# jeffreychou777/GenComm

Measured on AMD Instinct MI355X. Metric: scenes/sec, higher is better.
Workload: dtype f32

## Files before the change

gencomm_amd/csrc/conv8h8_kernels.h:

```cpp
#pragma once
#include "conv8h_kernels.h"
#include "split_f16.h"

namespace gc {

constexpr int H8_TH = 8, H8_LH = H8_TH + 2;
constexpr int H8_PLANE = H8_LH * HC_ROW;
constexpr int H8_TPLANE = H8_PLANE / 2;
constexpr int H8_TOFF = 2 * H8_PLANE;
constexpr int H8_TILE_BYTES = 2 * H8_PLANE + H8_TPLANE;

struct Tile8Regs {
  float4 v[8];
  float2 h;
};
template <bool GN>
__device__ __forceinline__ void h8_load(Tile8Regs& R, const float* __restrict__ sp, unsigned plane_in, int H, int W, int x0, int y0, int tid) {
  const int r0 = tid >> 4, qx = tid & 15;
  if (r0 < H8_LH) {
    const int gy = y0 - 1 + r0, gx = x0 + 4 * qx;
    if (GN) {
      const int cy = min(max(gy, 0), H - 1), cx = min(gx, W - 4);
#pragma unroll
      for (int c = 0; c < 8; ++c) R.v[c] = *reinterpret_cast<const float4*>(sp + ((unsigned)c * plane_in + (unsigned)cy * (unsigned)W + (unsigned)cx));
// ... 159 lines not shown
      for (int c = 0; c < 8; ++c) q = fmax(q, __hip_atomic_load(st + 2 * c + 1, __ATOMIC_RELAXED, __HIP_MEMORY_SCOPE_AGENT));
      bound = sqrtf((float)q) * 1.0001f;
    }
    mul = act_scale(bound);
  }
  const float inv_s = a.wh[NSRC * HC_WTAB3] / mul;
  const float4 bias4 = *reinterpret_cast<const float4*>(a.bias + 4 * ch);
  const float bias[4] = {bias4.x, bias4.y, bias4.z, bias4.w};
  Tile8Regs R;
  h8_load<GN>(R, a.src[0] + (size_t)n * 8 * plane, (unsigned)plane, a.H, a.W, x0, y0, tid);
  if (GN) {
    if (tid < NSRC * 8) {
      const int s = tid >> 3, c = tid & 7;
      float A, B;
      gn_coeff(a.sstat[s] + (size_t)n * 16, c, 2 * NSRC, a.inv_cnt, a.gamma[tid], a.beta[tid], &A, &B);
      s_ab[tid][0] = HC_NL2E * A;
      s_ab[tid][1] = HC_NL2E * B;
    }
    __syncthreads();
  }
  f32x4 acc[4];
  {
    const float sc = a.wh[NSRC * HC_WTAB3 + 1] * mul;
    const f32x4 b0 = {bias[0] * sc, bias[1] * sc, bias[2] * sc, bias[3] * sc};
#pragma unroll
    for (int j = 0; j < 4; ++j) acc[j] = b0;
  }
  h8_stage<GN>(tile, R, a.H, a.W, x0, y0, &s_ab[0], tid, mul);
  int off[4][3];
  h8_lane_offsets(off, wave, lane);
  float resv[RES == 1 ? 4 : 1][4];
  if (RES == 1 && wave_live) {
#pragma unroll
    for (int i = 0; i < 4; ++i) {
      const float* __restrict__ rp = a.res[0] + ((size_t)n * 8 + 4 * ch + i) * plane + (size_t)gy * a.W + gx;
      float4 r = make_float4(0.f, 0.f, 0.f, 0.f);
      if (vec_ok && gy < a.H) r = *reinterpret_cast<const float4*>(rp);
      resv[i][0] = r.x; resv[i][1] = r.y; resv[i][2] = r.z; resv[i][3] = r.w;
    }
  }
  if (NSRC == 2) h8_load<GN>(R, a.src[1] + (size_t)n * 8 * plane, (unsigned)plane, a.H, a.W, x0, y0, tid);
  __syncthreads();
  if (wave_live) h8_mfma3(tile, a.wh, acc, off, lane);
  if (NSRC == 2) {
    __syncthreads();
    h8_stage<GN>(tile, R, a.H, a.W, x0, y0, &s_ab[8], tid, 1.0f);
    __syncthreads();
    if (wave_live) h8_mfma3(tile, a.wh + HC_WTAB3, acc, off, lane);
  }
  float part[8];
#pragma unroll
  for (int i = 0; i < 8; ++i) part[i] = 0.f;
  if (wave_live) {
    float out[4][4];
#pragma unroll
    for (int i = 0; i < 4; ++i)
#pragma unroll
      for (int j = 0; j < 4; ++j) out[i][j] = RES == 1 ? fmaf(acc[j][i], inv_s, resv[i][j]) : acc[j][i] * inv_s;
    if (RES == 2) {
#pragma unroll 8
      for (int c = 0; c < 16; ++c) {
        const float4 wv4 = *reinterpret_cast<const float4*>(a.ninw + c * 8 + 4 * ch);
        const float wv[4] = {wv4.x, wv4.y, wv4.z, wv4.w};
        const float* __restrict__ rp = a.res[c >> 3] + ((size_t)n * 8 + (c & 7)) * plane + (size_t)gy * a.W + gx;
        float4 t = make_float4(0.f, 0.f, 0.f, 0.f);
        if (vec_ok && gy < a.H) t = *reinterpret_cast<const float4*>(rp);
        const float r[4] = {t.x, t.y, t.z, t.w};
#pragma unroll
        for (int i = 0; i < 4; ++i)
#pragma unroll
          for (int j = 0; j < 4; ++j) out[i][j] = fmaf(wv[i], r[j], out[i][j]);
      }
    }
#pragma unroll
    for (int i = 0; i < 4; ++i) {
      if (vec_ok && gy < a.H) {
        float* __restrict__ dp = a.dst + ((size_t)n * 8 + 4 * ch + i) * plane + (size_t)gy * a.W + gx;
        *reinterpret_cast<float4*>(dp) = make_float4(out[i][0], out[i][1], out[i][2], out[i][3]);
        float s = out[i][0] + out[i][1], q = out[i][0] * out[i][0];
        q = fmaf(out[i][1], out[i][1], q);
#pragma unroll
        for (int j = 2; j < 4; ++j) { s += out[i][j]; q = fmaf(out[i][j], out[i][j], q); }
        part[i] = s;
        part[4 + i] = q;
      }
    }
  }
  if (a.dstat != nullptr) hc_stats_commit(part, s_red, a.dstat + (size_t)n * 16, tid);
}

}
```

gencomm_amd/csrc/conv8h_kernels.h:

```cpp
#pragma once
#include "split_f16.h"
#include "unet_kernels.h"
#include "unet_plan.h"

namespace gc {

constexpr int HC_TW = 64, HC_TH = 16, HC_NT = 256, HC_LH = 18;
constexpr int HC_SLOTS = 18;
constexpr int HC_PHASE = HC_SLOTS * 16;
constexpr int HC_ROW = 4 * HC_PHASE;
constexpr int HC_PLANE = HC_LH * HC_ROW;
constexpr int HC_WTAB = 3 * 2 * 64 * 4;
constexpr int HC_WC3 = 3 * 64 * 4 + 64 * 2;
constexpr int HC_WTAB3 = 3 * HC_WC3;
static_assert(HC_WTAB3 == kWtab3, "unet_plan.h sizes the prepared blob with kWtab3");
constexpr int HC_TPLANE = HC_PLANE / 2;
constexpr int HC_TOFF = 2 * HC_PLANE;

constexpr float HC_NL2E = -1.4426950408889634f;
__device__ __forceinline__ void gn_silu_zr(float a2, float b2, float x, float& z, float& r, float cs = HC_NL2E) {
  z = fmaf(a2, x, b2);
  r = __builtin_amdgcn_rcpf(fmaf(cs, __builtin_amdgcn_exp2f(z), cs));
}
__device__ __forceinline__ int hc_addr(int row, int px ) {
// ... 390 lines not shown
    half8_t w[3];
#pragma unroll
    for (int k = 0; k < 3; ++k) w[k] = __builtin_bit_cast(half8_t, *reinterpret_cast<const uint4*>(tab + c * HC_WC3 + (k * 64 + lane) * 4));
#pragma unroll
    for (int p = 0; p < 2; ++p) {
      half8_t b[4];
#pragma unroll
      for (int j = 0; j < 4; ++j) b[j] = *reinterpret_cast<const half8_t*>(tile + off[j][c] + p * 2 * HC_ROW);
#pragma unroll
      for (int j = 0; j < 4; ++j) acc[p][j] = __builtin_amdgcn_mfma_f32_16x16x32_f16(w[2], b[j], acc[p][j], 0, 0, 0);
#pragma unroll
      for (int j = 0; j < 4; ++j) acc[p][j] = __builtin_amdgcn_mfma_f32_16x16x32_f16(w[1], b[j], acc[p][j], 0, 0, 0);
#pragma unroll
      for (int j = 0; j < 4; ++j) acc[p][j] = __builtin_amdgcn_mfma_f32_16x16x32_f16(w[0], b[j], acc[p][j], 0, 0, 0);
    }
  }
}

__device__ __forceinline__ void load_wa(half8_t (&wa)[3][2], const float* __restrict__ tab, int lane) {
#pragma unroll
  for (int c = 0; c < 3; ++c)
#pragma unroll
    for (int h = 0; h < 2; ++h) {
      const uint4 v = *reinterpret_cast<const uint4*>(tab + ((c * 2 + h) * 64 + lane) * 4);
      wa[c][h] = __builtin_bit_cast(half8_t, v);
    }
}

__device__ __forceinline__ void hc_stats_commit(float (&part)[8], float (*s_red)[16], double* __restrict__ dstat, int tid) {
  const int lane = tid & 63, wave = tid >> 6, ch = (lane >> 4) & 1;
#pragma unroll
  for (int v = 0; v < 8; ++v) {
    float x = part[v];
    x = dpp_add<0x111, 0xf>(x);
    x = dpp_add<0x112, 0xf>(x);
    x = dpp_add<0x114, 0xf>(x);
    x = dpp_add<0x118, 0xf>(x);
    x += __shfl_xor(x, 32, 64);
    part[v] = x;
  }
  if (lane == 15 || lane == 31) {
#pragma unroll
    for (int i = 0; i < 4; ++i) {
      s_red[wave][4 * ch + i] = part[i];
      s_red[wave][8 + 4 * ch + i] = part[4 + i];
    }
  }
  __syncthreads();
  if (tid < 16) {
    float v = 0.f;
#pragma unroll
    for (int w = 0; w < HC_NT / 64; ++w) v += s_red[w][tid];
    atomicAdd(&dstat[(tid & 7) * 2 + (tid >> 3)], (double)v);
  }
}

constexpr int HC_TILE_BYTES = 2 * HC_PLANE + HC_TPLANE;
struct HcCarry {
  TileRegs<HC_TW, HC_TH, HC_NT, 8> R;
  float2 hreg;
};
template <int NSRC, bool GN, bool UP, int RES, bool DIAG = false, bool PERSIST = false>
__device__ __forceinline__ void conv8h_tile(const Conv8Args& a, const BlockId bid, unsigned char* tile, float (*s_ab)[2], float (*s_red)[16],
                                            size_t bias_off, HcCarry& carry, bool have_next, const BlockId next) {
  constexpr int NT = HC_NT, TW = HC_TW, TH = HC_TH;
  TileRegs<TW, TH, NT, 8>& R = carry.R;
  float2& hreg = carry.hreg;
  fp16_ovfl_clamp();
  int tid_ = threadIdx.x;
  if (PERSIST) asm volatile("" : "+v"(tid_));
  const int tid = tid_, lane = tid & 63, wave = tid >> 6;
  const int n = bid.z;
  const int x0 = bid.x * TW, y0 = bid.y * TH;
  const size_t plane_in = (size_t)a.Hin * a.Win;
  const size_t plane = (size_t)a.H * a.W;
  const bool wvec = UP ? ((a.Win & 1) == 0) : ((a.W & 3) == 0);
  const int ln = lane & 15, g = lane >> 4, ch = g & 1, rr = g >> 1;
  const int gx = x0 + 4 * ln;
  const int gy0 = y0 + 4 * wave + rr;
  const bool vec_ok = (gx + 3 < a.W) && ((a.W & 3) == 0);
  const bool wave_live = y0 + 4 * wave < a.H;

  GC_STAMP(0);
  float mul = 1.0f;
  if (!GN) {
    float bound = 0.f;
    if (a.amax != nullptr) {
      bound = *a.amax;
    } else if (a.sstat[0] != nullptr) {
      const double* st = a.sstat[0] + (size_t)n * 16;
      double q = 0.0;
#pragma unroll
      for (int c = 0; c < 8; ++c) q = fmax(q, __hip_atomic_load(st + 2 * c + 1, __ATOMIC_RELAXED, __HIP_MEMORY_SCOPE_AGENT));
      bound = sqrtf((float)q) * 1.0001f;
    }
    mul = act_scale(bound);
  }
  const float inv_s = a.wh[NSRC * HC_WTAB3] / mul;
  const float4 bias4 = *reinterpret_cast<const float4*>(a.bias + bias_off + 4 * ch);
  const float bias[4] = {bias4.x, bias4.y, bias4.z, bias4.w};
  if (!PERSIST) {
    hreg = make_float2(0.f, 0.f);
    if (wvec) {
      stage_load<TW, TH, NT, 8, UP, GN>(R, a.src[0] + (size_t)n * 8 * plane_in, (unsigned)plane_in, a.Win, a.H, a.W, x0, y0, tid);
      hreg = halo_load_h<UP>(a.src[0] + (size_t)n * 8 * plane_in, (unsigned)plane_in, a.Win, a.H, a.W, x0, y0, tid);
    }
  }
  auto prefetch_next = [&]() {
    if (PERSIST && have_next) {
      const float* np = a.src[0] + (size_t)next.z * 8 * plane_in;
      stage_load<TW, TH, NT, 8, UP, GN>(R, np, (unsigned)plane_in, a.Win, a.H, a.W, next.x * TW, next.y * TH, tid);
      hreg = halo_load_h<UP>(np, (unsigned)plane_in, a.Win, a.H, a.W, next.x * TW, next.y * TH, tid);
    }
  };
  if (GN) {
    if (tid < NSRC * 8) {
      const int s = tid >> 3, c = tid & 7;
      float A, B;
      gn_coeff(a.sstat[s] + (size_t)n * 16, c, 2 * NSRC, a.inv_cnt, a.gamma[tid], a.beta[tid], &A, &B);
      s_ab[tid][0] = HC_NL2E * A;
      s_ab[tid][1] = HC_NL2E * B;
    }
    __syncthreads();
  }

  GC_STAMP(1);
  f32x4 acc[2][4];
  const float bsc = a.wh[NSRC * HC_WTAB3 + 1] * mul;
  const f32x4 b0 = {bias[0] * bsc, bias[1] * bsc, bias[2] * bsc, bias[3] * bsc};
  if (DIAG || !wave_live) {
#pragma unroll
    for (int p = 0; p < 2; ++p)
#pragma unroll
      for (int j = 0; j < 4; ++j) acc[p][j] = b0;
  }

  if (wvec) stage_store_h<GN, true>(tile, R, hreg, a.H, a.W, x0, y0, &s_ab[0], tid, mul);
  else stage_tile_scalar_h<GN, UP, true>(tile, a.src[0] + (size_t)n * 8 * plane_in, (unsigned)plane_in, a.Win, a.H, a.W, x0, y0, &s_ab[0], tid, mul);
  int off[4][3];
  hc_lane_offsets(off, wave, lane);
  float resv[RES == 1 ? 2 : 1][4][4];
  auto request_residual = [&]() {
  if (RES == 1 && wave_live) {
    const float* const lane_res = a.res[0] + ((size_t)n * 8 + 4 * ch) * plane + (size_t)gy0 * a.W + gx;
#pragma unroll
    for (int p = 0; p < 2; ++p)
#pragma unroll
      for (int i = 0; i < 4; ++i) {
        const int gy = gy0 + 2 * p;
        const float* __restrict__ rp = lane_res + ((size_t)i * plane + (size_t)(2 * p) * a.W);
        if (vec_ok && gy < a.H) {
          const float4 r = *reinterpret_cast<const float4*>(rp);
          resv[p][i][0] = r.x; resv[p][i][1] = r.y; resv[p][i][2] = r.z; resv[p][i][3] = r.w;
        } else {
#pragma unroll
          for (int j = 0; j < 4; ++j) resv[p][i][j] = (gy < a.H && gx + j < a.W) ? rp[j] : 0.f;
        }
      }
  }
  };
  constexpr bool LATE2 = PERSIST;
  auto early = [&]() {
    if (!PERSIST) request_residual();
    if (NSRC == 2 && wvec && !LATE2) {
      stage_load<TW, TH, NT, 8, UP, GN>(R, a.src[1] + (size_t)n * 8 * plane_in, (unsigned)plane_in, a.Win, a.H, a.W, x0, y0, tid);
      hreg = halo_load_h<UP>(a.src[1] + (size_t)n * 8 * plane_in, (unsigned)plane_in, a.Win, a.H, a.W, x0, y0, tid);
    }
  };
#ifdef HC_EARLY_IN_FRONT
  early();
#endif
  __syncthreads();
  GC_STAMP(2);
#ifdef HC_PRIO_MFMA
  __builtin_amdgcn_s_setprio(HC_PRIO_MFMA);
#endif
#ifdef HC_EARLY_IN_FRONT
  if (wave_live) conv_tile_mfma3<DIAG, NSRC == 2 && (!LATE2 || PERSIST), !DIAG>(tile, a.wh, acc, off, lane, a.term_mask, b0);
#else
  if (wave_live) conv_tile_mfma3<DIAG, NSRC == 2 && (!LATE2 || PERSIST), !DIAG>(tile, a.wh, acc, off, lane, a.term_mask, b0, early);
  else early();
#endif
  if (NSRC == 2 && wvec && LATE2) {
    stage_load<TW, TH, NT, 8, UP, GN>(R, a.src[1] + (size_t)n * 8 * plane_in, (unsigned)plane_in, a.Win, a.H, a.W, x0, y0, tid);
    hreg = halo_load_h<UP>(a.src[1] + (size_t)n * 8 * plane_in, (unsigned)plane_in, a.Win, a.H, a.W, x0, y0, tid);
  }
  if (DIAG && (a.term_mask & 128) && wave_live) conv_tile_mfma3<DIAG, NSRC == 2>(tile, a.wh, acc, off, lane, a.term_mask);
  GC_STAMP(3);
  if (NSRC == 2) {
    __syncthreads();
    if (wvec) stage_store_h<GN, true>(tile, R, hreg, a.H, a.W, x0, y0, &s_ab[8], tid);
    else stage_tile_scalar_h<GN, UP, true>(tile, a.src[1] + (size_t)n * 8 * plane_in, (unsigned)plane_in, a.Win, a.H, a.W, x0, y0, &s_ab[8], tid);
    __syncthreads();
    if (wave_live) conv_tile_mfma3<false, PERSIST>(tile, a.wh + HC_WTAB3, acc, off, lane);
  }

  if (PERSIST) request_residual();
  if (RES != 2) prefetch_next();
  GC_STAMP(4);
#ifdef HC_PRIO_EPI
  __builtin_amdgcn_s_setprio(HC_PRIO_EPI);
#endif
  float part[8];
#pragma unroll
  for (int i = 0; i < 8; ++i) part[i] = 0.f;
  if (wave_live) {
    float* const lane_dst = a.dst + ((size_t)n * 8 + 4 * ch) * plane + (size_t)gy0 * a.W + gx;
    float out[2][4][4];
#pragma unroll
    for (int p = 0; p < 2; ++p)
#pragma unroll
      for (int i = 0; i < 4; ++i)
#pragma unroll
        for (int j = 0; j < 4; ++j) out[p][i][j] = RES == 1 ? fmaf(acc[p][j][i], inv_s, resv[p][i][j]) : acc[p][j][i] * inv_s;

    if (RES == 2) {
      const size_t lane_off = (size_t)n * 8 * plane;
      if ((a.W & 3) == 0) {
        int gxl = gx, gyl = gy0;
        asm volatile("" : "+v"(gxl), "+v"(gyl));
        const int cx = min(gxl, a.W - 4);
        const int cy0 = min(gyl, a.H - 1), d1 = (min(gyl + 2, a.H - 1) - cy0) * a.W;
        const size_t o0 = lane_off + (size_t)cy0 * a.W + cx;
        const float* const lp[2][2] = {{a.res[0] + o0, a.res[0] + o0 + d1}, {a.res[1] + o0, a.res[1] + o0 + d1}};
        constexpr int CB = 4;
        float4 rq[2][CB][2];
        auto issue = [&](int b, int st) {
#pragma unroll
          for (int c = 0; c < CB; ++c)
#pragma unroll
            for (int p = 0; p < 2; ++p) {
              const int cc = b * CB + c;
              rq[st][c][p] = *reinterpret_cast<const float4*>(lp[cc >> 3][p] + (size_t)(cc & 7) * plane);
            }
        };
        issue(0, 0);
#pragma unroll
        for (int b = 0; b < 16 / CB; ++b) {
          __builtin_amdgcn_sched_barrier(0);
          if (b + 1 < 16 / CB) issue(b + 1, (b + 1) & 1);
#pragma unroll
          for (int c = 0; c < CB; ++c) {
            const float4 wv4 = *reinterpret_cast<const float4*>(a.ninw + (b * CB + c) * 8 + 4 * ch);
            const float wv[4] = {wv4.x, wv4.y, wv4.z, wv4.w};
#pragma unroll
            for (int p = 0; p < 2; ++p) {
              const float4 t = rq[b & 1][c][p];
              const float r[4] = {t.x, t.y, t.z, t.w};
#pragma unroll
              for (int i = 0; i < 4; ++i)
#pragma unroll
                for (int j = 0; j < 4; ++j) out[p][i][j] = fmaf(wv[i], r[j], out[p][i][j]);
            }
          }
        }
      } else {
#pragma unroll 1
        for (int c = 0; c < 16; ++c) {
          const float4 wv4 = *reinterpret_cast<const float4*>(a.ninw + c * 8 + 4 * ch);
          const float wv[4] = {wv4.x, wv4.y, wv4.z, wv4.w};
#pragma unroll
          for (int p = 0; p < 2; ++p) {
            const int gy = gy0 + 2 * p;
            const float* __restrict__ rp = a.res[c >> 3] + ((size_t)n * 8 + (c & 7)) * plane + (size_t)gy * a.W + gx;
            float r[4];
#pragma unroll
            for (int j = 0; j < 4; ++j) r[j] = (gy < a.H && gx + j < a.W) ? rp[j] : 0.f;
#pragma unroll
            for (int i = 0; i < 4; ++i)
#pragma unroll
              for (int j = 0; j < 4; ++j) out[p][i][j] = fmaf(wv[i], r[j], out[p][i][j]);
          }
        }
      }
    }

    if (RES == 2) prefetch_next();
#pragma unroll
    for (int p = 0; p < 2; ++p) {
      const int gy = gy0 + 2 * p;
#pragma unroll
      for (int i = 0; i < 4; ++i) {
        float* __restrict__ dp = lane_dst + ((size_t)i * plane + (size_t)(2 * p) * a.W);
        float s = 0.f, q = 0.f;
        if (vec_ok && gy < a.H) {
          if (!(DIAG && (a.term_mask & 64)))
            *reinterpret_cast<float4*>(dp) = make_float4(out[p][i][0], out[p][i][1], out[p][i][2], out[p][i][3]);
          s = out[p][i][0] + out[p][i][1];
          q = out[p][i][0] * out[p][i][0];
          q = fmaf(out[p][i][1], out[p][i][1], q);
#pragma unroll
          for (int j = 2; j < 4; ++j) { s += out[p][i][j]; q = fmaf(out[p][i][j], out[p][i][j], q); }
        } else {
#pragma unroll
          for (int j = 0; j < 4; ++j)
            if (gy < a.H && gx + j < a.W) { dp[j] = out[p][i][j]; s += out[p][i][j]; q = fmaf(out[p][i][j], out[p][i][j], q); }
        }
        part[i] = p == 0 ? s : part[i] + s;
        part[4 + i] = p == 0 ? q : part[4 + i] + q;
      }
    }
  } else if (RES == 2) {
    prefetch_next();
  }
  GC_STAMP(5);
  if (a.dstat != nullptr) hc_stats_commit(part, s_red, a.dstat + (size_t)n * 16, tid);
  GC_STAMP(6);
  if (PERSIST) __syncthreads();
}
template <int NSRC, bool GN, bool UP, int RES, bool DIAG = false>
__device__ __forceinline__ void conv8h_tile(const Conv8Args& a, const BlockId bid, unsigned char* tile, float (*s_ab)[2], float (*s_red)[16],
                                            size_t bias_off = 0) {
  HcCarry carry;
  conv8h_tile<NSRC, GN, UP, RES, DIAG, false>(a, bid, tile, s_ab, s_red, bias_off, carry, false, bid);
}

template <int NSRC, bool GN, bool UP, int RES, bool DIAG = false>
__global__ __launch_bounds__(HC_NT, 3) void conv8h_kernel(const Conv8Args a) {
  __shared__ __align__(16) unsigned char tile[HC_TILE_BYTES];
  __shared__ float s_ab[16][2];
  __shared__ float s_red[HC_NT / 64][16];
#ifdef HC_LDS_PAD
  __shared__ float s_pad[HC_LDS_PAD / 4];
  if (a.H < 0) s_pad[threadIdx.x] = 1.f;
#endif
  conv8h_tile<NSRC, GN, UP, RES, DIAG>(a, xcd_block(a.xcd), tile, s_ab, s_red);
}

template <int NSRC, bool GN, bool UP, int RES>
__global__ __launch_bounds__(HC_NT, 3) void conv8hp_kernel(const Conv8Args a, int tx, int ty, int nz) {
// ... 7 lines not shown
  BlockId bid = xcd_block_dims(a.xcd, lin, (unsigned)tx, (unsigned)ty, total);
  HcCarry carry;
  {
    const float* sp = a.src[0] + (size_t)bid.z * 8 * plane_in;
    stage_load<HC_TW, HC_TH, HC_NT, 8, UP, GN>(carry.R, sp, (unsigned)plane_in, a.Win, a.H, a.W, bid.x * HC_TW, bid.y * HC_TH, threadIdx.x);
    carry.hreg = halo_load_h<UP>(sp, (unsigned)plane_in, a.Win, a.H, a.W, bid.x * HC_TW, bid.y * HC_TH, threadIdx.x);
  }
#pragma unroll 1
  for (; lin < total; lin += gridDim.x) {
    const unsigned nl = lin + gridDim.x;
    const bool have_next = nl < total;
    const BlockId nb = have_next ? xcd_block_dims(a.xcd, nl, (unsigned)tx, (unsigned)ty, total) : bid;
    conv8h_tile<NSRC, GN, UP, RES, false, true>(a, bid, tile, s_ab, s_red, 0, carry, have_next, nb);
    bid = nb;
  }
}

__global__ __launch_bounds__(256) void prep_conv8h_kernel(const float* __restrict__ w, float* __restrict__ dst, int IC) {
  const int tid = threadIdx.x;
  float m = 0.f;
  for (int i = tid; i < 8 * IC * 9; i += 256) m = fmaxf(m, fabsf(w[i]));
  const float scale = block_weight_scale(m);
  const int nsrc = IC / 8;
  uint32_t* __restrict__ out = reinterpret_cast<uint32_t*>(dst);
  auto weight = [&](int s, int c, int l, int ch) -> float {
    const int mrow = l & 15, kg = l >> 4, r = mrow >> 3, oc = mrow & 7;
    const int dyp = hc_tap_row(kg), dx = c, dy = dyp - r;
    return (dy >= 0 && dy <= 2) ? w[((oc * IC + s * 8 + ch) * 3 + dy) * 3 + dx] * scale : 0.f;
  };
  for (int i = tid; i < nsrc * HC_WTAB3; i += 256) {
    const int s = i / HC_WTAB3, rem = i - s * HC_WTAB3;
    const int c = rem / HC_WC3, q = rem - c * HC_WC3;
    if (q < 768) {
      const int d = q & 3, l = (q >> 2) & 63, term = q >> 8;
      uint16_t v[2];
      for (int e = 0; e < 2; ++e) {
        const float x = weight(s, c, l, 2 * d + e);
        const _Float16 w1 = (_Float16)x;
        const float r1 = x - (float)w1;
        const _Float16 w2 = (_Float16)r1;
        const _Float16 w3 = (_Float16)(r1 - (float)w2);
        v[e] = __builtin_bit_cast(uint16_t, term == 0 ? w1 : term == 1 ? w2 : w3);
      }
      out[i] = (uint32_t)v[0] | ((uint32_t)v[1] << 16);
    } else {
      const int d = (q - 768) & 1, l = (q - 768) >> 1;
      const float k = 1.0f / HC_TSCALE;
      out[i] = bf8x4(weight(s, c, l, 4 * d) * k, weight(s, c, l, 4 * d + 1) * k, weight(s, c, l, 4 * d + 2) * k, weight(s, c, l, 4 * d + 3) * k);
    }
  }
  if (tid < 64) dst[nsrc * HC_WTAB3 + tid] = (tid & 1) ? scale : 1.0f / scale;
}

}
```

gencomm_amd/csrc/unet_host.h:

```cpp
#pragma once
#include <stdlib.h>

#include "attn_kernels.h"
#include "conv8b_kernels.h"
#include "conv8h_kernels.h"
#include "conv8h8_kernels.h"
#include "dataflow_kernels.h"
#include "latent_kernels.h"
#include "latenth_kernels.h"
#include "unet_kernels.h"
#include "unet_plan.h"

namespace gc {

inline int cdiv(int a, int b) { return (a + b - 1) / b; }

enum TileCfg { TILE_64x16 = 0, TILE_32x16 = 1, TILE_32x8 = 2 };
inline long long tile_want(const Modes& m) {
  return m.v[MODE_TILE_WANT] > 0 ? m.v[MODE_TILE_WANT] : (m.split() ? 160LL : 512LL);
}
inline TileCfg pick_tile(const Modes& m, int n, int H, int W, int zmul = 1) {
  if (m.bf16()) return TILE_64x16;
  const long long want = tile_want(m);
  if ((long long)cdiv(W, 64) * cdiv(H, 16) * n * zmul >= want) return TILE_64x16;
// ... 58 lines not shown
}

template <int NSRC, bool GN, bool UP, int RES>
inline void launch_conv8b(const Conv8BArgs& a, int n, hipStream_t st) {
  const double elt = 2.0;
  const double abytes = elt * n * ((double)NSRC * 8 * a.Hin * a.Win + (RES == 1 ? 8.0 : RES == 2 ? 16.0 : 0.0) * a.H * a.W + 8.0 * a.H * a.W);
  TimedLaunch tl(UP ? KF_UP : (NSRC == 2 ? KF_CONV16 : (RES == 1 ? KF_CONV8_RES1 : RES == 2 ? KF_CONV8_RES2 : KF_CONV8)), st, abytes);
  GC_KLOG("conv8b_kernel<...> (bf16 storage)");
  conv8b_kernel<NSRC, GN, UP, RES><<<dim3(cdiv(a.W, 64), cdiv(a.H, 16), n), 256, 0, st>>>(a);
}

struct UNetCall {
  const UNetPlan* plan;
  const UNetWorkspace* ws;
  const float* prepared;
  char* wsp;
  int n, H, W;
  hipStream_t st;
  Modes m;
  float* amax() const { return reinterpret_cast<float*>(wsp + ws->amax_off); }
  int is_f32(int id) const { return (!m.bf16() || id == plan->hs0_tensor) ? 1 : 0; }

  float* tensor_ptr(int id) const {
    const TensorPlan& t = plan->tensors[id];
    return reinterpret_cast<float*>(wsp + ws->level_base[t.level] + ws->slot_bytes[t.level] * t.slot);
  }
  double* stat_ptr(int id) const { return reinterpret_cast<double*>(wsp) + (size_t)id * n * 16; }
};

inline Conv8Args conv1_args(const UNetCall& c, const Op& o, int t) {
  const ResBlockPlan& b = c.plan->blocks[o.blk];
  const float* P = c.prepared;
  const int Hl = c.ws->Hl[o.level], Wl = c.ws->Wl[o.level];
  Conv8Args a{};
  a.src[0] = c.tensor_ptr(o.src[0]); a.sstat[0] = c.stat_ptr(o.src[0]);
  if (o.src[1] >= 0) { a.src[1] = c.tensor_ptr(o.src[1]); a.sstat[1] = c.stat_ptr(o.src[1]); }
  a.gamma = P + b.n1w; a.beta = P + b.n1b;
  a.w = P + b.p_c1w; a.wh = P + b.p_c1wh; a.bias = P + b.p_bias1 + (size_t)t * 8;
  a.dst = c.tensor_ptr(o.dst); a.dstat = c.stat_ptr(o.dst);
  a.H = a.Hin = Hl; a.W = a.Win = Wl;
  a.inv_cnt = 1.0 / ((b.cin == 8 ? 2.0 : 4.0) * Hl * Wl);
  a.xcd = c.m.xcd();
  return a;
}
inline Conv8Args conv2_args(const UNetCall& c, const Op& o) {
  const ResBlockPlan& b = c.plan->blocks[o.blk];
  const float* P = c.prepared;
  const int Hl = c.ws->Hl[o.level], Wl = c.ws->Wl[o.level];
  Conv8Args a{};
  a.src[0] = c.tensor_ptr(o.src[0]); a.sstat[0] = c.stat_ptr(o.src[0]);
  a.gamma = P + b.n2w; a.beta = P + b.n2b;
  a.w = P + b.p_c2w; a.wh = P + b.p_c2wh; a.bias = P + b.p_bias2;
  a.res[0] = c.tensor_ptr(o.res[0]);
  if (o.res[1] >= 0) { a.res[1] = c.tensor_ptr(o.res[1]); a.ninw = P + b.p_ninw; }
  a.dst = c.tensor_ptr(o.dst); a.dstat = c.stat_ptr(o.dst);
  a.H = a.Hin = Hl; a.W = a.Win = Wl;
  a.inv_cnt = 1.0 / (2.0 * Hl * Wl);
  a.xcd = c.m.xcd();
  return a;
}
inline Conv8Args up_args(const UNetCall& c, const Op& o) {
  const UNetPlan& p = *c.plan;
  const float* P = c.prepared;
  const int lin = o.level + 1;
  Conv8Args a{};
  a.src[0] = c.tensor_ptr(o.src[0]);
  a.sstat[0] = c.stat_ptr(o.src[0]);
  a.w = P + p.up[lin].p_w; a.wh = P + p.up[lin].p_wh; a.bias = P + p.up[lin].b;
  a.dst = c.tensor_ptr(o.dst); a.dstat = c.stat_ptr(o.dst);
  a.H = c.ws->Hl[o.level]; a.W = c.ws->Wl[o.level]; a.Hin = c.ws->Hl[lin]; a.Win = c.ws->Wl[lin];
  a.xcd = c.m.xcd();
  return a;
}
inline DownArgs down_args(const UNetCall& c, const Op& o) {
  const UNetPlan& p = *c.plan;
  const float* P = c.prepared;
  const int lin = o.level - 1;
  return DownArgs{c.tensor_ptr(o.src[0]), P + p.down[lin].p_w, P + p.down[lin].b, c.tensor_ptr(o.dst), c.stat_ptr(o.dst),
                  c.ws->Hl[o.level], c.ws->Wl[o.level], c.ws->Hl[lin], c.ws->Wl[lin], !c.is_f32(o.src[0]), !c.is_f32(o.dst)};
}

inline bool resfuse_emulated(const UNetCall& c, const ResBlockPlan& b, TileCfg tc, bool wvec) {
  return c.m.v[MODE_RESFUSE_EMU] != 0 && b.cin == 8 && tc == TILE_64x16 && c.m.split() && !c.m.bf16() && wvec;
}

inline bool df_eligible(const UNetCall& c, int f, int l) {
  if (c.m.v[MODE_DATAFLOW] == 0 || !c.m.split() || c.m.bf16() || l - f < 2 || l - f > DF_MAX_OPS || c.n > 64 * 1024) return false;
  if (c.m.v[MODE_CONV8H_MASK] != -1) return false;
  for (int oi = f; oi < l; ++oi) {
    const Op& o = c.plan->ops[oi];
    if (o.kind != OP_RES_CONV1 && o.kind != OP_RES_CONV2 && o.kind != OP_DOWN && o.kind != OP_UP) return false;
    if (o.kind == OP_DOWN) {
      if ((c.ws->Wl[o.level - 1] & 3) != 0) return false;
    } else if (pick_tile(c.m, c.n, c.ws->Hl[o.level], c.ws->Wl[o.level]) != TILE_64x16) return false;
  }
  return true;
}
inline int df_enqueue(const UNetCall& c, int t, int f, int l, bool upload) {
  const UNetPlan& p = *c.plan;
  DfProgram* dprog = reinterpret_cast<DfProgram*>(c.wsp + c.ws->df_prog_off);
  unsigned* words = reinterpret_cast<unsigned*>(c.wsp + c.ws->df_words_off);
  const int nops = l - f;
  if (upload) {
    static thread_local DfProgram hp;
    hp.nops = nops; hp.n = c.n;
    int qlen[8] = {0, 0, 0, 0, 0, 0, 0, 0};
    for (int k = 0; k < nops; ++k) {
// ... 249 lines not shown
  a.a_bf16 = !c.is_f32(p.last_body_tensor);
  TimedLaunch tl(KF_LATENT_STEP, c.st, 4.0 * c.n * 32.0 * c.H * c.W);
  const bool small_h = c.m.split() && (c.W & 3) == 0 && c.W >= 64 && c.H >= 16 && c.m.v[MODE_TILE_WANT] == 0;
  if ((pick_tile(c.m, c.n, c.H, c.W) == TILE_64x16 || small_h) && c.m.split()) {
    const dim3 grid(cdiv(c.W, 64), cdiv(c.H, 16), c.n);
    GC_KLOG(noise ? "latent_step_h_kernel<1> (explicit noise)" : "latent_step_h_kernel<2> (in-kernel Philox)");
    if (noise) latent_step_h_kernel<1><<<grid, 256, 0, c.st>>>(a);
    else latent_step_h_kernel<2><<<grid, 256, 0, c.st>>>(a);
  } else if (pick_tile(c.m, c.n, c.H, c.W) == TILE_64x16) {
    const dim3 grid(cdiv(c.W, 64), cdiv(c.H, 16), c.n);
    GC_KLOG(noise ? "latent_step_kernel<64,16,1> (exact fp32, explicit noise)" : "latent_step_kernel<64,16,2> (exact fp32, in-kernel Philox)");
    if (noise) latent_step_kernel<64, 16, 1><<<grid, 256, 0, c.st>>>(a);
    else latent_step_kernel<64, 16, 2><<<grid, 256, 0, c.st>>>(a);
  } else {
    const dim3 grid(cdiv(c.W, 32), cdiv(c.H, 16), c.n);
    GC_KLOG(noise ? "latent_step_kernel<32,16,1> (exact fp32, explicit noise)" : "latent_step_kernel<32,16,2> (exact fp32, in-kernel Philox)");
    if (noise) latent_step_kernel<32, 16, 1><<<grid, 128, 0, c.st>>>(a);
    else latent_step_kernel<32, 16, 2><<<grid, 128, 0, c.st>>>(a);
  }
  GC_HIP(hipGetLastError());
  return GC_OK;
}

inline int unet_prepare_enqueue(const UNetPlan& p, const float* raw, float* prepared, hipStream_t st) {
  GC_HIP(hipMemcpyAsync(prepared, raw, (size_t)p.raw_floats * sizeof(float), hipMemcpyDeviceToDevice, st));
  auto conv_w = [&](long long src, long long dst, int OC, int IC, int OCB) {
    const int total = OC * IC * 9;
    prep_conv_w_kernel<<<cdiv(total, 256), 256, 0, st>>>(raw + src, prepared + dst, OC, IC, OCB);
  };
  conv_w(p.conv_in.w, p.conv_in.p_w, 8, p.C + 2, 8);
  GC_HIP(hipMemsetAsync(prepared + p.conv_out.p_w, 0, (size_t)((p.C + 15) / 16 * 16) * 72 * sizeof(float), st));
  conv_w(p.conv_out.w, p.conv_out.p_w, p.C, 8, 16);
  prep_conv_out_h_kernel<<<1, 256, 0, st>>>(raw + p.conv_out.w, prepared + p.conv_out.p_wh, p.C);
  for (int l = 0; l < p.L; ++l) {
    if (p.down[l].w >= 0) conv_w(p.down[l].w, p.down[l].p_w, 8, 8, 8);
    if (p.up[l].w >= 0) {
      conv_w(p.up[l].w, p.up[l].p_w, 8, 8, 8);
      prep_conv8h_kernel<<<1, 256, 0, st>>>(raw + p.up[l].w, prepared + p.up[l].p_wh, 8);
      prep_conv8b_kernel<<<1, 256, 0, st>>>(raw + p.up[l].w, prepared + p.up[l].p_wb, 8);
    }
  }
  TembArgs ta{};
  ta.raw = raw; ta.prepared = prepared;
  ta.d0w = p.d0w; ta.d0b = p.d0b; ta.d1w = p.d1w; ta.d1b = p.d1b;
  ta.nblocks = (int)p.blocks.size(); ta.T = p.T;
  for (size_t i = 0; i < p.blocks.size(); ++i) {
    const ResBlockPlan& b = p.blocks[i];
    conv_w(b.c1w, b.p_c1w, 8, b.cin, 8);
    conv_w(b.c2w, b.p_c2w, 8, 8, 8);
    prep_conv8h_kernel<<<1, 256, 0, st>>>(raw + b.c1w, prepared + b.p_c1wh, b.cin);
    prep_conv8h_kernel<<<1, 256, 0, st>>>(raw + b.c2w, prepared + b.p_c2wh, 8);
    prep_conv8b_kernel<<<1, 256, 0, st>>>(raw + b.c1w, prepared + b.p_c1wb, b.cin);
    prep_conv8b_kernel<<<1, 256, 0, st>>>(raw + b.c2w, prepared + b.p_c2wb, 8);
    if (b.cin != 8) prep_nin_w_kernel<<<1, 256, 0, st>>>(raw + b.ninw, prepared + b.p_ninw, 8, b.cin);
    prep_add_kernel<<<1, 64, 0, st>>>(raw + b.c2b, b.cin != 8 ? raw + b.ninb : nullptr, prepared + b.p_bias2, 8);
    ta.tpw[i] = b.tpw; ta.tpb[i] = b.tpb; ta.c1b[i] = b.c1b; ta.dst[i] = b.p_bias1;
  }
  prep_temb_kernel<<<p.T, 64, 0, st>>>(ta);
  {
    PrepLatentArgs la{raw + p.conv_in.w, raw + p.conv_out.w, raw + p.conv_out.b, prepared + p.p_wc5, prepared + p.p_wc1,
                      prepared + p.p_bring, prepared + p.p_bsum, p.C};
    prep_latent_kernel<<<cdiv(1600 + 5184 + 72 + 8, 256), 256, 0, st>>>(la);
    prep_latent_h_kernel<<<1, 256, 0, st>>>(prepared + p.p_wc5, raw + p.conv_in.w, prepared + p.p_wc5h, prepared + p.p_wxh,
                                           prepared + p.p_wch, p.C);
  }
  GC_HIP(hipGetLastError());
  return GC_OK;
}

}
```

gencomm_amd/csrc/unet_kernels.h:

```cpp
#pragma once
#include <type_traits>

#include "common.h"

namespace gc {

__device__ __forceinline__ void gn_coeff(const double* __restrict__ stat ,
                                         int c, int gs, double inv_cnt, float gamma, float beta,
                                         float* A, float* B) {
  const int g0 = c & ~(gs - 1);
  double s = 0.0, q = 0.0;
  for (int j = 0; j < gs; ++j) {
    s += stat[(g0 + j) * 2 + 0];
    q += stat[(g0 + j) * 2 + 1];
  }
  const double mean = s * inv_cnt;
  const float var = fmaxf((float)(q * inv_cnt - mean * mean), 0.f);
  const float rstd = __builtin_amdgcn_rsqf(var + 1e-6f);
  const float a = gamma * rstd;
  *A = a;
  *B = beta - (float)mean * a;
}

template <int NT>
// ... 181 lines not shown
    constexpr int ic = decltype(IC)::value;
    float in[3][PPL + 2];
#pragma unroll
    for (int dy = 0; dy < 3; ++dy) {
      if constexpr (PPL == 4) {
        const float4 v = *reinterpret_cast<const float4*>(&tile[ic][ty + dy][tx * 4 + 4]);
        in[dy][0] = tile[ic][ty + dy][tx * 4 + 3];
        in[dy][1] = v.x; in[dy][2] = v.y; in[dy][3] = v.z; in[dy][4] = v.w;
        in[dy][5] = tile[ic][ty + dy][tx * 4 + 8];
      } else {
        in[dy][0] = tile[ic][ty + dy][tx + 3];
        in[dy][1] = tile[ic][ty + dy][tx + 4];
        in[dy][2] = tile[ic][ty + dy][tx + 5];
      }
    }
    static_for<0, 9>([&](auto TAP) {
      constexpr int tap = decltype(TAP)::value, dy = tap / 3, dx = tap % 3;
      static_for<0, NOG>([&](auto OG) {
        constexpr int og = decltype(OG)::value;
        constexpr int f = (ic * 9 + tap) * NOG + og;
#pragma unroll
        for (int p = 0; p < PPL; ++p) acc[og][p] = mfma_wbcast<f % 16>(wr[f / 16], in[dy][p + dx], acc[og][p]);
      });
    });
  });
}

__device__ __forceinline__ void gn_mean_rstd(const double* __restrict__ stat, int c, int gs, double inv_cnt, float* mean, float* rstd) {
  const int g0 = c & ~(gs - 1);
  double s = 0.0, q = 0.0;
  for (int j = 0; j < gs; ++j) { s += stat[(g0 + j) * 2 + 0]; q += stat[(g0 + j) * 2 + 1]; }
  const double m = s * inv_cnt;
  const float var = fmaxf((float)(q * inv_cnt - m * m), 0.f);
  *mean = (float)m;
  *rstd = __builtin_amdgcn_rsqf(var + 1e-6f);
}

__device__ __forceinline__ float silu_grad_f(float z) {
  const float s = sigmoid_f(z);
  return s * fmaf(z, 1.0f - s, 1.0f);
}


struct Conv8Args {
  const float* src[2];
  const double* sstat[2];
  const float* gamma;
  const float* beta;
  const float* w;
  const float* wh;
  const float* bias;
  const float* res[2];
  const float* ninw;
  float* dst;
  double* dstat;
  double inv_cnt;
  int H, W, Hin, Win;
  int xcd;
  const float* amax;
  int term_mask;
  int gn_gs;
  int src_ct, dst_ct;
};

template <int TW, int TH, int PPL, int NSRC, bool GN, bool UP, int RES>
__global__ __launch_bounds__((TW / PPL) * TH) void conv8_kernel(const Conv8Args a) {
  constexpr int NT = (TW / PPL) * TH;
  constexpr int LH = TH + 2, LS = TW + 8;
  static_assert(NT % 64 == 0, "workgroup must be whole waves");
  __shared__ __align__(16) float tile[8][LH][LS];
  __shared__ float s_ab[16][2];
  __shared__ float s_red[NT / 64][16];

  const int tid = threadIdx.x, lane = tid & 63;
  const BlockId bid = xcd_block(a.xcd);
  const int n = bid.z;
  const int x0 = bid.x * TW, y0 = bid.y * TH;
  const int tx = tid % (TW / PPL), ty = tid / (TW / PPL);
  const size_t plane_in = (size_t)a.Hin * a.Win;
  const size_t src_ns = (size_t)(a.src_ct ? a.src_ct : 8) * plane_in;
  const size_t plane = (size_t)a.H * a.W;
  const bool wvec = UP ? ((a.Win & 1) == 0) : ((a.W & 3) == 0);
  const int gy = y0 + ty, gx = x0 + tx * PPL;
  const bool row_ok = gy < a.H;
  const bool vec_ok = PPL == 4 && row_ok && (gx + 3 < a.W) && ((a.W & 3) == 0);
  bool ok[PPL];
#pragma unroll
  for (int p = 0; p < PPL; ++p) ok[p] = row_ok && (gx + p < a.W);
  const size_t pix = (size_t)gy * a.W + gx;
  constexpr int ROWS_PER_WAVE = 64 / (TW / PPL);
  const bool wave_live = y0 + (tid >> 6) * ROWS_PER_WAVE < a.H;

  GC_STAMP(0);
  float wr[NSRC][9];
#pragma unroll
  for (int s = 0; s < NSRC; ++s) load_wregs<9>(wr[s], a.w + s * 576, 576, lane);
  float bias[8];
#pragma unroll
  for (int o = 0; o < 8; ++o) bias[o] = as_const(a.bias)[o];
  TileRegs<TW, TH, NT, 8> R;
  if (GC_EXP & 16) R = TileRegs<TW, TH, NT, 8>{};
  else if (wvec) stage_load<TW, TH, NT, 8, UP>(R, a.src[0] + (size_t)n * src_ns, (unsigned)plane_in, a.Win, a.H, a.W, x0, y0, tid);
  float resv[(RES == 1 || RES == 3) ? 8 : 1][PPL];
  if (RES == 1 || RES == 3) {
#pragma unroll
    for (int o = 0; o < 8; ++o) {
// ... 575 lines not shown
```

gencomm_amd/csrc/unet_plan.h:

```cpp
#pragma once
#include <string>
#include <vector>

#include "common.h"

namespace gc {

constexpr int kWtab3 = 3 * (3 * 64 * 4 + 64 * 2);

struct ParamEntry {
  std::string name;
  long long numel;
  long long off;
};

struct ResBlockPlan {
  int cin;
  long long n1w, n1b, c1w, c1b, tpw, tpb, n2w, n2b, c2w, c2b, ninw, ninb;
  long long p_c1w, p_c2w, p_ninw, p_bias1 , p_bias2 ;
  long long p_c1wh, p_c2wh;
  long long p_c1wb, p_c2wb;
};

struct AttnPlan {
  long long nw, nb, qw, qb, kw, kb, vw, vb, pw, pb;
};

struct ConvPlan {
  long long w, b;
  long long p_w;
  long long p_wh = -1;
  long long p_wb = -1;
};

enum OpKind { OP_CONV_IN, OP_RES_CONV1, OP_RES_CONV2, OP_DOWN, OP_UP, OP_CONV_OUT, OP_ATTN };

struct Op {
  OpKind kind;
  int blk;
  int src[2];
  int res[2];
  int dst;
  int level;
};

struct TensorPlan {
  int level;
  int slot;
  int last_use;
};

struct UNetPlan {
  int C, L, R, T, attn_mask;
  std::vector<AttnPlan> attns;
  std::vector<ParamEntry> params;
  long long raw_floats = 0;
  long long prepared_floats = 0;
  long long d0w, d0b, d1w, d1b;
  ConvPlan conv_in, conv_out;
  long long nout_w, nout_b;
  long long p_wc5, p_wc1, p_bring, p_bsum;
  long long p_wc5h, p_wxh, p_wch;
  int hs0_tensor = 0, last_body_tensor = 0;
  std::vector<ConvPlan> down, up;
  std::vector<ResBlockPlan> blocks;
  std::vector<Op> ops;
  std::vector<TensorPlan> tensors;
  std::vector<int> slots_per_level;

  long long add(const std::string& name, long long numel) {
    params.push_back({name, numel, raw_floats});
    const long long o = raw_floats;
    raw_floats += numel;
    return o;
// ... 70 lines not shown
    d0b = add("temb.dense.0.bias", 32);
    d1w = add("temb.dense.1.weight", 32 * 32);
    d1b = add("temb.dense.1.bias", 32);
    conv_in.w = add("conv_in.weight", 8LL * (C + 2) * 9);
    conv_in.b = add("conv_in.bias", 8);
    std::vector<std::vector<int>> down_blk(L), up_blk(L), down_att(L), up_att(L);
    for (int l = 0; l < L; ++l) {
      for (int b = 0; b < R; ++b) {
        down_blk[l].push_back(add_resblock("down." + std::to_string(l) + ".block." + std::to_string(b), 8));
        if (attn_mask >> l & 1) down_att[l].push_back(add_attn("down." + std::to_string(l) + ".attn." + std::to_string(b)));
      }
      if (l != L - 1) {
        down[l].w = add("down." + std::to_string(l) + ".downsample.conv.weight", 8 * 8 * 9);
        down[l].b = add("down." + std::to_string(l) + ".downsample.conv.bias", 8);
      }
    }
    const int mid1 = add_resblock("mid.block_1", 8), mid2 = add_resblock("mid.block_2", 8);
    for (int l = L - 1; l >= 0; --l) {
      for (int b = 0; b <= R; ++b) {
        up_blk[l].push_back(add_resblock("up." + std::to_string(l) + ".block." + std::to_string(b), 16));
        if (attn_mask >> l & 1) up_att[l].push_back(add_attn("up." + std::to_string(l) + ".attn." + std::to_string(b)));
      }
      if (l != 0) {
        up[l].w = add("up." + std::to_string(l) + ".upsample.conv.weight", 8 * 8 * 9);
        up[l].b = add("up." + std::to_string(l) + ".upsample.conv.bias", 8);
      }
    }
    nout_w = add("norm_out.weight", 8);
    nout_b = add("norm_out.bias", 8);
    conv_out.w = add("conv_out.weight", (long long)C * 8 * 9);
    conv_out.b = add("conv_out.bias", C);
    if ((int)blocks.size() > kMaxResBlocks) return "too many res-blocks";

    prepared_floats = (raw_floats + 63) / 64 * 64;
    conv_in.p_w = padd(8LL * (C + 2) * 9);
    conv_out.p_w = padd((long long)((C + 15) / 16 * 16) * 8 * 9);
    conv_out.p_wh = padd((long long)((C + 15) / 16) * kWtab3 + 64);
    for (int l = 0; l < L; ++l) {
      if (down[l].w >= 0) down[l].p_w = padd(8 * 8 * 9);
      if (up[l].w >= 0) { up[l].p_w = padd(8 * 8 * 9); up[l].p_wh = padd(kWtab3 + 64); up[l].p_wb = padd(768); }
    }
    p_wc5 = padd(1600); p_wc1 = padd(5184); p_bring = padd(72); p_bsum = padd(8);
    p_wc5h = padd(8 * (kWtab3 / 3) + 64); p_wxh = padd((long long)(C / 8) * kWtab3); p_wch = padd(kWtab3);
    for (auto& b : blocks) {
      b.p_c1w = padd(8LL * b.cin * 9);
      b.p_c2w = padd(8 * 8 * 9);
      b.p_ninw = b.cin != 8 ? padd(8LL * b.cin) : -1;
      b.p_bias1 = padd((long long)T * 8);
      b.p_bias2 = padd(8);
      b.p_c1wh = padd((long long)(b.cin / 8) * kWtab3 + 64);
      b.p_c2wh = padd(kWtab3 + 64);
      b.p_c1wb = padd((long long)(b.cin / 8) * 768);
      b.p_c2wb = padd(768);
    }

    std::vector<int> hs;
    int h = new_tensor(0);
    ops.push_back({OP_CONV_IN, 0, {-1, -1}, {-1, -1}, h, 0});
    hs.push_back(h);
    for (int l = 0; l < L; ++l) {
      for (int b = 0; b < R; ++b) {
        int t = emit_resblock(down_blk[l][b], hs.back(), -1, l);
        if (attn_mask >> l & 1) t = emit_attn(down_att[l][b], t, l);
        hs.push_back(t);
      }
      if (l != L - 1) {
        const int d = new_tensor(l + 1);
        ops.push_back({OP_DOWN, l, {hs.back(), -1}, {-1, -1}, d, l + 1});
        hs.push_back(d);
      }
    }
    h = hs.back();
    h = emit_resblock(mid1, h, -1, L - 1);
    h = emit_resblock(mid2, h, -1, L - 1);
    for (int l = L - 1; l >= 0; --l) {
      for (int b = 0; b <= R; ++b) {
        const int skip = hs.back();
        hs.pop_back();
        h = emit_resblock(up_blk[l][b], h, skip, l);
        if (attn_mask >> l & 1) h = emit_attn(up_att[l][b], h, l);
      }
      if (l != 0) {
        const int u = new_tensor(l - 1);
        ops.push_back({OP_UP, l, {h, -1}, {-1, -1}, u, l - 1});
        h = u;
      }
    }
    ops.push_back({OP_CONV_OUT, 0, {h, -1}, {-1, -1}, -1, 0});
    hs0_tensor = ops[0].dst;
    last_body_tensor = h;

    for (int i = 0; i < (int)ops.size(); ++i) {
      const Op& o = ops[i];
      for (int k = 0; k < 2; ++k) {
        if (o.src[k] >= 0) tensors[o.src[k]].last_use = i;
        if (o.res[k] >= 0) tensors[o.res[k]].last_use = i;
      }
    }
    tensors[hs0_tensor].last_use = (int)ops.size();
    slots_per_level.assign(L, 0);
    std::vector<std::vector<int>> free_slots(L);
    auto take_slot = [&](int id) {
      TensorPlan& t = tensors[id];
      if (!free_slots[t.level].empty()) {
        t.slot = free_slots[t.level].back();
        free_slots[t.level].pop_back();
// ... 57 lines not shown
```

Before: 189.2.

## Compute nin 1x1 shortcut with split-precision MFMA instead of scalar FMAs

Replaces the scalar 16-channel 1x1 nin shortcut in the residual conv epilogue with an MFMA path. It splits activations into f16 hi/lo plus a bf8 tail and multiplies them against a prepared weight table, scaling by a bound derived from the residual tensors' statistics. A new prep kernel builds the table, and plan and args gain offsets for it and for the residual stat pointers. The goal is to offload the FMA-heavy shortcut to matrix cores and overlap next-tile prefetch with it. This adds precision-emulation error risk and extra stat reads.

Result: no change. 189.9, median of 3 (+0.4%).

```diff
diff --git a/gencomm_amd/csrc/conv8h8_kernels.h b/gencomm_amd/csrc/conv8h8_kernels.h
--- a/gencomm_amd/csrc/conv8h8_kernels.h
+++ b/gencomm_amd/csrc/conv8h8_kernels.h
@@ -235,35 +235,24 @@
 #pragma unroll
   for (int i = 0; i < 8; ++i) part[i] = 0.f;
   if (wave_live) {
-    float out[4][4];
+    float out[1][4][4];
 #pragma unroll
     for (int i = 0; i < 4; ++i)
 #pragma unroll
-      for (int j = 0; j < 4; ++j) out[i][j] = RES == 1 ? fmaf(acc[j][i], inv_s, resv[i][j]) : acc[j][i] * inv_s;
+      for (int j = 0; j < 4; ++j) out[0][i][j] = RES == 1 ? fmaf(acc[j][i], inv_s, resv[i][j]) : acc[j][i] * inv_s;
     if (RES == 2) {
-#pragma unroll 8
-      for (int c = 0; c < 16; ++c) {
-        const float4 wv4 = *reinterpret_cast<const float4*>(a.ninw + c * 8 + 4 * ch);
-        const float wv[4] = {wv4.x, wv4.y, wv4.z, wv4.w};
-        const float* __restrict__ rp = a.res[c >> 3] + ((size_t)n * 8 + (c & 7)) * plane + (size_t)gy * a.W + gx;
-        float4 t = make_float4(0.f, 0.f, 0.f, 0.f);
-        if (vec_ok && gy < a.H) t = *reinterpret_cast<const float4*>(rp);
-        const float r[4] = {t.x, t.y, t.z, t.w};
-#pragma unroll
-        for (int i = 0; i < 4; ++i)
-#pragma unroll
-          for (int j = 0; j < 4; ++j) out[i][j] = fmaf(wv[i], r[j], out[i][j]);
-      }
+      const float* const lp = (ch ? a.res[1] : a.res[0]) + (size_t)n * 8 * plane + (size_t)min(gy, a.H - 1) * a.W + min(gx, a.W - 4);
+      hc_nin_shortcut<1>(a.wh + a.ninwh_off, a.sstat[0] + a.rstat_off[0] + (size_t)n * 16, a.sstat[0] + a.rstat_off[1] + (size_t)n * 16, lp, 0, plane, lane, out);
     }
 #pragma unroll
     for (int i = 0; i < 4; ++i) {
       if (vec_ok && gy < a.H) {
         float* __restrict__ dp = a.dst + ((size_t)n * 8 + 4 * ch + i) * plane + (size_t)gy * a.W + gx;
-        *reinterpret_cast<float4*>(dp) = make_float4(out[i][0], out[i][1], out[i][2], out[i][3]);
-        float s = out[i][0] + out[i][1], q = out[i][0] * out[i][0];
-        q = fmaf(out[i][1], out[i][1], q);
-#pragma unroll
-        for (int j = 2; j < 4; ++j) { s += out[i][j]; q = fmaf(out[i][j], out[i][j], q); }
+        *reinterpret_cast<float4*>(dp) = make_float4(out[0][i][0], out[0][i][1], out[0][i][2], out[0][i][3]);
+        float s = out[0][i][0] + out[0][i][1], q = out[0][i][0] * out[0][i][0];
+        q = fmaf(out[0][i][1], out[0][i][1], q);
+#pragma unroll
+        for (int j = 2; j < 4; ++j) { s += out[0][i][j]; q = fmaf(out[0][i][j], out[0][i][j], q); }
         part[i] = s;
         part[4 + i] = q;
       }
diff --git a/gencomm_amd/csrc/conv8h_kernels.h b/gencomm_amd/csrc/conv8h_kernels.h
--- a/gencomm_amd/csrc/conv8h_kernels.h
+++ b/gencomm_amd/csrc/conv8h_kernels.h
@@ -466,6 +466,87 @@
 #pragma unroll
     for (int w = 0; w < HC_NT / 64; ++w) v += s_red[w][tid];
     atomicAdd(&dstat[(tid & 7) * 2 + (tid >> 3)], (double)v);
+  }
+}
+
+constexpr int HC_NINTAB = HC_WC3;
+static_assert(HC_NINTAB == kWtab3 / 3, "unet_plan.h sizes the prepared blob with kWtab3 / 3");
+template <int NP, bool AHEAD = false, class AfterLoads = HcNoEarly>
+__device__ __forceinline__ void hc_nin_shortcut(const float* __restrict__ tab, const double* __restrict__ st0, const double* __restrict__ st1,
+                                                const float* __restrict__ lp, int d1, size_t plane, int lane, float (&out)[NP][4][4],
+                                                AfterLoads after_loads = AfterLoads()) {
+  const int sc = lane & 15;
+  float q = (float)__hip_atomic_load((sc & 8 ? st1 : st0) + 2 * (sc & 7) + 1, __ATOMIC_RELAXED, __HIP_MEMORY_SCOPE_AGENT);
+  WA3 wa;
+  load_wa3(wa, tab, 0, lane);
+  float4 raw[NP][8];
+  auto request = [&](int p) {
+#pragma unroll
+    for (int c = 0; c < 8; ++c) raw[p][c] = *reinterpret_cast<const float4*>(lp + (size_t)c * plane + (size_t)(p * d1));
+  };
+  request(0);
+  if (AHEAD && NP > 1) request(1);
+#pragma unroll
+  for (int k = 1; k < 16; k <<= 1) q = fmaxf(q, __shfl_xor(q, k, 64));
+  const float mul = act_scale(sqrtf(q) * 1.0001f);
+  const float inv_ns = tab[HC_NINTAB] / mul;
+#pragma unroll
+  for (int p = 0; p < NP; ++p) {
+    half8_t bh[4], bl[4];
+    long bt[4];
+    {
+      float e[8][4];
+#pragma unroll
+      for (int c = 0; c < 8; ++c) { e[c][0] = raw[p][c].x; e[c][1] = raw[p][c].y; e[c][2] = raw[p][c].z; e[c][3] = raw[p][c].w; }
+      if (mul != 1.0f) {
+#pragma unroll
+        for (int c = 0; c < 8; ++c)
+#pragma unroll
+          for (int j = 0; j < 4; ++j) e[c][j] *= mul;
+      }
+#pragma unroll
+      for (int j = 0; j < 4; ++j) {
+        uint4 hi, lo;
+        float t[8];
+        split3_pair(e[0][j], e[1][j], hi.x, lo.x, t[0], t[1]);
+        split3_pair(e[2][j], e[3][j], hi.y, lo.y, t[2], t[3]);
+        split3_pair(e[4][j], e[5][j], hi.z, lo.z, t[4], t[5]);
+        split3_pair(e[6][j], e[7][j], hi.w, lo.w, t[6], t[7]);
+        bh[j] = __builtin_bit_cast(half8_t, hi);
+        bl[j] = __builtin_bit_cast(half8_t, lo);
+        bt[j] = __builtin_bit_cast(long, make_uint2(bf8x4s(t[0], t[1], t[2], t[3]), bf8x4s(t[4], t[5], t[6], t[7])));
+      }
+    }
+    constexpr int FENCE = 0x2 | 0x4;
+    f32x4 s[4];
+    if (p == NP - 1) after_loads();
+    __builtin_amdgcn_sched_barrier(FENCE);
+#pragma unroll
+    for (int j = 0; j < 4; ++j) {
+      s[j] = __builtin_amdgcn_mfma_f32_16x16x32_bf8_bf8(wa.wb, bt[j], (f32x4{0.f, 0.f, 0.f, 0.f}), 0, 0, 0);
+      __builtin_amdgcn_sched_barrier(FENCE);
+    }
+#pragma unroll
+    for (int j = 0; j < 4; ++j) {
+      s[j] = __builtin_amdgcn_mfma_f32_16x16x32_f16(wa.w[2], bh[j], s[j], 0, 0, 0);
+      __builtin_amdgcn_sched_barrier(FENCE);
+    }
+#pragma unroll
+    for (int j = 0; j < 4; ++j) s[j] = __builtin_amdgcn_mfma_f32_16x16x32_f16(wa.w[1], bl[j], s[j], 0, 0, 0);
+#pragma unroll
+    for (int j = 0; j < 4; ++j) s[j] = __builtin_amdgcn_mfma_f32_16x16x32_f16(wa.w[1], bh[j], s[j], 0, 0, 0);
+#pragma unroll
+    for (int j = 0; j < 4; ++j) s[j] = __builtin_amdgcn_mfma_f32_16x16x32_f16(wa.w[0], bl[j], s[j], 0, 0, 0);
+    __builtin_amdgcn_sched_barrier(FENCE);
+    if (!AHEAD && p + 1 < NP) request(p + 1);
+    __builtin_amdgcn_sched_barrier(FENCE);
+#pragma unroll
+    for (int j = 0; j < 4; ++j) s[j] = __builtin_amdgcn_mfma_f32_16x16x32_f16(wa.w[0], bh[j], s[j], 0, 0, 0);
+    __builtin_amdgcn_sched_barrier(FENCE);
+#pragma unroll
+    for (int i = 0; i < 4; ++i)
+#pragma unroll
+      for (int j = 0; j < 4; ++j) out[p][i][j] = fmaf(s[j][i], inv_ns, out[p][i][j]);
   }
 }
 
@@ -525,6 +606,9 @@
       const float* np = a.src[0] + (size_t)next.z * 8 * plane_in;
       stage_load<TW, TH, NT, 8, UP, GN>(R, np, (unsigned)plane_in, a.Win, a.H, a.W, next.x * TW, next.y * TH, tid);
       hreg = halo_load_h<UP>(np, (unsigned)plane_in, a.Win, a.H, a.W, next.x * TW, next.y * TH, tid);
+    } else if (PERSIST && RES == 2) {
+      R = TileRegs<TW, TH, NT, 8>{};
+      hreg = make_float2(0.f, 0.f);
     }
   };
   if (GN) {
@@ -630,44 +714,15 @@
 
     if (RES == 2) {
       const size_t lane_off = (size_t)n * 8 * plane;
-      if ((a.W & 3) == 0) {
+      if (PERSIST || (a.W & 3) == 0) {
         int gxl = gx, gyl = gy0;
+        size_t pl = plane;
         asm volatile("" : "+v"(gxl), "+v"(gyl));
+        if constexpr (PERSIST) asm volatile("" : "+s"(pl));
         const int cx = min(gxl, a.W - 4);
         const int cy0 = min(gyl, a.H - 1), d1 = (min(gyl + 2, a.H - 1) - cy0) * a.W;
-        const size_t o0 = lane_off + (size_t)cy0 * a.W + cx;
-        const float* const lp[2][2] = {{a.res[0] + o0, a.res[0] + o0 + d1}, {a.res[1] + o0, a.res[1] + o0 + d1}};
-        constexpr int CB = 4;
-        float4 rq[2][CB][2];
-        auto issue = [&](int b, int st) {
-#pragma unroll
-          for (int c = 0; c < CB; ++c)
-#pragma unroll
-            for (int p = 0; p < 2; ++p) {
-              const int cc = b * CB + c;
-              rq[st][c][p] = *reinterpret_cast<const float4*>(lp[cc >> 3][p] + (size_t)(cc & 7) * plane);
-            }
-        };
-        issue(0, 0);
-#pragma unroll
-        for (int b = 0; b < 16 / CB; ++b) {
-          __builtin_amdgcn_sched_barrier(0);
-          if (b + 1 < 16 / CB) issue(b + 1, (b + 1) & 1);
-#pragma unroll
-          for (int c = 0; c < CB; ++c) {
-            const float4 wv4 = *reinterpret_cast<const float4*>(a.ninw + (b * CB + c) * 8 + 4 * ch);
-            const float wv[4] = {wv4.x, wv4.y, wv4.z, wv4.w};
-#pragma unroll
-            for (int p = 0; p < 2; ++p) {
-              const float4 t = rq[b & 1][c][p];
-              const float r[4] = {t.x, t.y, t.z, t.w};
-#pragma unroll
-              for (int i = 0; i < 4; ++i)
-#pragma unroll
-                for (int j = 0; j < 4; ++j) out[p][i][j] = fmaf(wv[i], r[j], out[p][i][j]);
-            }
-          }
-        }
+        const float* const lp = (ch ? a.res[1] : a.res[0]) + lane_off + (size_t)cy0 * a.W + cx;
+        hc_nin_shortcut<2, !PERSIST>(a.wh + a.ninwh_off, a.sstat[0] + a.rstat_off[0] + (size_t)n * 16, a.sstat[0] + a.rstat_off[1] + (size_t)n * 16, lp, d1, pl, lane, out, prefetch_next);
       } else {
 #pragma unroll 1
         for (int c = 0; c < 16; ++c) {
@@ -686,10 +741,10 @@
               for (int j = 0; j < 4; ++j) out[p][i][j] = fmaf(wv[i], r[j], out[p][i][j]);
           }
         }
-      }
-    }
-
-    if (RES == 2) prefetch_next();
+        prefetch_next();
+      }
+    }
+
 #pragma unroll
     for (int p = 0; p < 2; ++p) {
       const int gy = gy0 + 2 * p;
@@ -803,4 +858,17 @@
   if (tid < 64) dst[nsrc * HC_WTAB3 + tid] = (tid & 1) ? scale : 1.0f / scale;
 }
 
-}
+__global__ __launch_bounds__(256) void prep_nin_h_kernel(const float* __restrict__ w, float* __restrict__ dst) {
+  const int tid = threadIdx.x;
+  const float scale = block_weight_scale(tid < 128 ? fabsf(w[tid]) : 0.f);
+  uint32_t* __restrict__ out = reinterpret_cast<uint32_t*>(dst);
+  for (int q = tid; q < HC_NINTAB; q += 256) {
+    const int l = wtab_lane(q), m = l & 15, kg = l >> 4;
+    float wv[8];
+    for (int e = 0; e < 8; ++e) wv[e] = (m >> 3) == (kg >> 1) ? w[(m & 7) * 16 + 8 * (kg & 1) + e] * scale : 0.f;
+    out[q] = wtab_entry(q, wv);
+  }
+  if (tid < 64) dst[HC_NINTAB + tid] = (tid & 1) ? scale : 1.0f / scale;
+}
+
+}
diff --git a/gencomm_amd/csrc/unet_host.h b/gencomm_amd/csrc/unet_host.h
--- a/gencomm_amd/csrc/unet_host.h
+++ b/gencomm_amd/csrc/unet_host.h
@@ -134,7 +134,10 @@
   a.gamma = P + b.n2w; a.beta = P + b.n2b;
   a.w = P + b.p_c2w; a.wh = P + b.p_c2wh; a.bias = P + b.p_bias2;
   a.res[0] = c.tensor_ptr(o.res[0]);
-  if (o.res[1] >= 0) { a.res[1] = c.tensor_ptr(o.res[1]); a.ninw = P + b.p_ninw; }
+  if (o.res[1] >= 0) {
+    a.res[1] = c.tensor_ptr(o.res[1]); a.ninw = P + b.p_ninw; a.ninwh_off = (int)(b.p_ninwh - b.p_c2wh);
+    for (int k = 0; k < 2; ++k) a.rstat_off[k] = (int)(c.stat_ptr(o.res[k]) - a.sstat[0]);
+  }
   a.dst = c.tensor_ptr(o.dst); a.dstat = c.stat_ptr(o.dst);
   a.H = a.Hin = Hl; a.W = a.Win = Wl;
   a.inv_cnt = 1.0 / (2.0 * Hl * Wl);
@@ -490,7 +493,10 @@
     prep_conv8h_kernel<<<1, 256, 0, st>>>(raw + b.c2w, prepared + b.p_c2wh, 8);
     prep_conv8b_kernel<<<1, 256, 0, st>>>(raw + b.c1w, prepared + b.p_c1wb, b.cin);
     prep_conv8b_kernel<<<1, 256, 0, st>>>(raw + b.c2w, prepared + b.p_c2wb, 8);
-    if (b.cin != 8) prep_nin_w_kernel<<<1, 256, 0, st>>>(raw + b.ninw, prepared + b.p_ninw, 8, b.cin);
+    if (b.cin != 8) {
+      prep_nin_w_kernel<<<1, 256, 0, st>>>(raw + b.ninw, prepared + b.p_ninw, 8, b.cin);
+      prep_nin_h_kernel<<<1, 256, 0, st>>>(raw + b.ninw, prepared + b.p_ninwh);
+    }
     prep_add_kernel<<<1, 64, 0, st>>>(raw + b.c2b, b.cin != 8 ? raw + b.ninb : nullptr, prepared + b.p_bias2, 8);
     ta.tpw[i] = b.tpw; ta.tpb[i] = b.tpb; ta.c1b[i] = b.c1b; ta.dst[i] = b.p_bias1;
   }
diff --git a/gencomm_amd/csrc/unet_kernels.h b/gencomm_amd/csrc/unet_kernels.h
--- a/gencomm_amd/csrc/unet_kernels.h
+++ b/gencomm_amd/csrc/unet_kernels.h
@@ -257,6 +257,8 @@
   const float* bias;
   const float* res[2];
   const float* ninw;
+  int ninwh_off;
+  int rstat_off[2];
   float* dst;
   double* dstat;
   double inv_cnt;
diff --git a/gencomm_amd/csrc/unet_plan.h b/gencomm_amd/csrc/unet_plan.h
--- a/gencomm_amd/csrc/unet_plan.h
+++ b/gencomm_amd/csrc/unet_plan.h
@@ -20,6 +20,7 @@
   long long p_c1w, p_c2w, p_ninw, p_bias1 , p_bias2 ;
   long long p_c1wh, p_c2wh;
   long long p_c1wb, p_c2wb;
+  long long p_ninwh;
 };
 
 struct AttnPlan {
@@ -196,6 +197,7 @@
       b.p_c2wh = padd(kWtab3 + 64);
       b.p_c1wb = padd((long long)(b.cin / 8) * 768);
       b.p_c2wb = padd(768);
+      b.p_ninwh = b.cin != 8 ? padd(kWtab3 / 3 + 64) : -1;
     }
 
     std::vector<int> hs;
```
